# duckietown/gym-duckietown

Hardware: NVIDIA H100
Metric: env-steps/sec (obs+reward+done) at N envs, 1/2/4/8 H100 vs CPU ref (higher is better)
Workload: dtype f64 logic / f32 raster / u8 obs

## Files before the change

### gym-duckietown_b200/csrc/dts_render.cu

```cuda
#include <algorithm>
#include <cstddef>
#include <cstdlib>
#include <iterator>
#include <type_traits>
#include <utility>
#include <vector>

#include "dts_camera.cuh"
#include "dts_kernels.h"

namespace dts {

struct RemapTab {
  const int32_t* src_xy;
  const short4* cbox;
  const short4* fbox;
  const int32_t* cell_start;
  const uint16_t* cell_bins;
  const int32_t* home_start;
  const int4* home_ent;
  int ext_x, ext_y;
  const uint16_t* table_of_env;
  int count;
  const float2* fwd;
// ... 532 lines not shown
  }
  if (cls_out) *cls_out = 0;
  if (ltq & 0x00ff0000) {
    const unsigned ti = si.tex;
    const int lw = (ti >> 24) & 15, lh = ti >> 28;
    const int tw = 1 << lw, th = 1 << lh;
    const float twf = __int_as_float((127 + lw) << 23), thf = __int_as_float((127 + lh) << 23);
    const float tx = u * twf - 0.5f, ty = v * thf - 0.5f;
    const int txi = __float2int_rd(tx), tyi = __float2int_rd(ty);
    const float ffx = tx - (float)txi, ffy = ty - (float)tyi;
    const unsigned ti0 = (unsigned)txi & (tw - 1), ti1 = (ti0 + 1) & (tw - 1);
    const unsigned tj0 = (unsigned)tyi & (th - 1), tj1 = (tj0 + 1) & (th - 1);
    const unsigned r0 = tj0 << lw, r1 = tj1 << lw;
    const uchar4* tp = reinterpret_cast<const uchar4*>(tex_pool + ((size_t)(ti & 0xffffffu) << 8));
    const uchar4 t00 = __ldg(tp + (r0 + ti0)), t10 = __ldg(tp + (r0 + ti1));
    const uchar4 t01 = __ldg(tp + (r1 + ti0)), t11 = __ldg(tp + (r1 + ti1));
    const float a0[3] = {(float)t00.x, (float)t00.y, (float)t00.z}, a1[3] = {(float)t10.x, (float)t10.y, (float)t10.z};
    const float b0[3] = {(float)t01.x, (float)t01.y, (float)t01.z}, b1[3] = {(float)t11.x, (float)t11.y, (float)t11.z};
#pragma unroll
    for (int ch = 0; ch < 3; ch++) {
      const float ta = fmaf(ffx, a1[ch] - a0[ch], a0[ch]);
      const float tb = fmaf(ffx, b1[ch] - b0[ch], b0[ch]);
      const float tc = fmaf(ffy, tb - ta, ta);
      c3[ch] = tc * (c3[ch] * 0.00392156862745098f);
    }
    if (cls_out) {
      const unsigned cu = (unsigned)__float2int_rd(u * twf) & (tw - 1), cv = (unsigned)__float2int_rd(v * thf) & (th - 1);
      *cls_out = __ldg(cls_pool + ((size_t)(ti & 0xffffffu) << 6) + ((cv << lw) + cu));
    }
  }
}
__device__ __forceinline__ void shade_prim(const PrimRec* __restrict__ prims, unsigned w, const uint8_t* __restrict__ tex_pool,
                                           const float4* __restrict__ lat_tab, int pxa, int pya, float c3[3], float* qq_out = nullptr,
                                           const uint8_t* __restrict__ cls_pool = nullptr, int* cls_out = nullptr) {
  const ShadeIn si = load_shade(prims, w);
  shade_eval(si, tex_pool, lat_tab, pxa, pya, c3, qq_out, cls_pool, cls_out);
}

__device__ __forceinline__ uint32_t smem_u32(const void* p) { return (uint32_t)__cvta_generic_to_shared(p); }
__device__ __forceinline__ void mbar_init(uint64_t* bar, int count) {
  asm volatile("mbarrier.init.shared::cta.b64 [%0], %1;" ::"r"(smem_u32(bar)), "r"(count) : "memory");
}
__device__ __forceinline__ void mbar_fence_init() {
  asm volatile("fence.mbarrier_init.release.cluster;" ::: "memory");
  asm volatile("fence.proxy.async.shared::cta;" ::: "memory");
}
__device__ __forceinline__ void mbar_expect_tx(uint64_t* bar, uint32_t bytes) {
  asm volatile("mbarrier.arrive.expect_tx.shared::cta.b64 _, [%0], %1;" ::"r"(smem_u32(bar)), "r"(bytes) : "memory");
}
__device__ __forceinline__ void bulk_load(void* dst_smem, const void* src_gmem, uint32_t bytes, uint64_t* bar) {
  asm volatile("cp.async.bulk.shared::cluster.global.mbarrier::complete_tx::bytes [%0], [%1], %2, [%3];" ::"r"(smem_u32(dst_smem)),
               "l"(src_gmem), "r"(bytes), "r"(smem_u32(bar))
               : "memory");
}
__device__ __forceinline__ void mbar_wait(uint64_t* bar, uint32_t parity) {
  uint32_t ok;
  do {
    asm volatile("{\n .reg .pred p;\n mbarrier.try_wait.parity.shared::cta.b64 p, [%1], %2;\n selp.u32 %0, 1, 0, p;\n}"
                 : "=r"(ok)
                 : "r"(smem_u32(bar)), "r"(parity)
                 : "memory");
  } while (!ok);
}

__device__ __forceinline__ unsigned pack_rgb(float r, float g, float b) {
  const unsigned ur = min(__float2uint_rn(r * 255.0f), 255u);
  const unsigned ug = min(__float2uint_rn(g * 255.0f), 255u);
  const unsigned ub = min(__float2uint_rn(b * 255.0f), 255u);
  return ur | (ug << 8) | (ub << 16);
}

struct StoreLane {
  int src_lo, src_hi;
  int sh8;
  int off;
  int j, row;
};
__device__ __forceinline__ StoreLane make_store_lane(int lane, int W) {
  StoreLane sl;
  const int j = lane & 7, rowbase = lane & ~7;
  const int p0 = (4 * j) / 3;
  sl.sh8 = (4 * j - 3 * p0) * 8;
  sl.src_lo = rowbase + min(p0, 7);
  sl.src_hi = rowbase + min(p0 + 1, 7);
  sl.off = (lane >> 3) * W * 3 + 4 * j;
  sl.j = j; sl.row = lane >> 3;
  return sl;
}
__device__ __forceinline__ void store_bin_fast(uint8_t* __restrict__ bin0, const StoreLane& sl, unsigned rgb, int rows_ok) {
  const unsigned lo = __shfl_sync(0xffffffffu, rgb, sl.src_lo);
  const unsigned hi = __shfl_sync(0xffffffffu, rgb, sl.src_hi);
  const unsigned word = __funnelshift_r(lo | (hi << 24), hi >> 8, sl.sh8);
  if (sl.j < 6 && sl.row < rows_ok) *reinterpret_cast<unsigned*>(bin0 + sl.off) = word;
}
__device__ __forceinline__ void store_bin_bytes(uint8_t* __restrict__ out, unsigned rgb, int lane, int bx, int by, int W, int H) {
  const int gx = bx * kBinW + (lane & 7), gy = by * kBinH + (lane >> 3);
  if (gx < W && gy < H) {
    uint8_t* d = out + ((size_t)gy * W + gx) * 3;
    d[0] = (uint8_t)(rgb & 255); d[1] = (uint8_t)((rgb >> 8) & 255); d[2] = (uint8_t)(rgb >> 16);
  }
}

__device__ __forceinline__ unsigned fine_rows_in_image(int cby, int H) { return ((cby * kCFY + 1) * kBinH < H) ? 0xffu : 0x0fu; }
__device__ __forceinline__ unsigned fine_in_image(int cbx, unsigned rows, int W) {
  const int nx = min(kCFX, (W - cbx * kCoarseW + kBinW - 1) / kBinW);
  const unsigned cols = (1u << nx) - 1u;
// ... 642 lines not shown
  __syncthreads();
  BinRec* recs = fm.recs;
  for (int i = pair0 + tid; i < pair0 + total; i += nthr) {
    const uint32_t pair = pairs[i];
    const int p = (int)(pair & 0xffffu), b = (int)(pair >> 16);
    const int cby = b / cbins_x, cbx = b - cby * cbins_x;
    unsigned r;
    if (kRemap != kRemapNone) {
      const short4 cb = rt.cbox[b];
      r = build_binrec(prims + p, p, cb.x * kSub, cb.y * kSub, recs + i, rt.fbox + (size_t)b * 8);
    } else {
      r = build_binrec(prims + p, p, cbx * kCoarseW * kSub, cby * kCoarseH * kSub, recs + i);
    }
    const int c = cnt[b];
    const unsigned valid = fine_in_image(cbx, fine_rows_in_image(cby, H), W);
    const bool alone = (r & kRecGround) ? (c & kCountMask) == 1 : (c & kCountMask) - (c >> 20) == 1;
    if (alone && (r & valid) == valid) {
      fm.bin_count[(size_t)env * cbins + b] = -(p + 1);
      const int slot = atomicAdd(fm.work + kWorkSoloList, 1);
      fm.solo[slot] = make_uint2((unsigned)env, (unsigned)b | ((unsigned)p << 16));
      atomicOr(&no_flat[b], 1 | kSoloMark);
    }
    if (!(r & kRecFlatOk)) atomicOr(&no_flat[b], 1);
  }
  __syncthreads();
  for (int b0 = wib * 32; b0 < cbins; b0 += nthr) {
    const int b = b0 + lane, c = b < cbins ? (cnt[b] & kCountMask) : 0;
    const bool flat = c >= 1 && c <= kStage && !no_flat[b];
    const bool empty = kRemap == kRemapNone && (W & 3) == 0 && b < cbins && c == 0;
    const unsigned m = __ballot_sync(0xffffffffu, flat), me = __ballot_sync(0xffffffffu, empty);
    if (m) {
      int base = 0;
      if (lane == 0) base = atomicAdd(fm.work + kWorkFlatList, __popc(m));
      base = __shfl_sync(0xffffffffu, base, 0);
      if (flat) {
        fm.bin_count[(size_t)env * cbins + b] = kFlatBin;
        fm.flat[base + __popc(m & ((1u << lane) - 1u))] = make_uint2((unsigned)env, (unsigned)b | ((unsigned)c << 16));
      }
    }
    if (me) {
      DTS_COUNT(30, __popc(me));
      int base = 0;
      if (lane == 0) base = atomicAdd(fm.work + kWorkEmptyList, __popc(me));
      base = __shfl_sync(0xffffffffu, base, 0);
      if (empty) {
        fm.bin_count[(size_t)env * cbins + b] = kEmptyBin;
        fm.empty[base + __popc(me & ((1u << lane) - 1u))] = make_uint2((unsigned)env, (unsigned)b);
      }
    }
    if (b < cbins && (rc.all_rows || (!flat && !empty && !(no_flat[b] & kSoloMark)))) row_to_list(fm, env, b / cbins_x, cbins_y);
  }
}

__device__ __noinline__ void gather_rows_out(const uint8_t* __restrict__ src, const GatherTab& gt, size_t off, size_t nbytes, int lane) {
  __syncwarp();
  const uint8_t* s = src + off;
  if (((reinterpret_cast<size_t>(s) | nbytes) & 15) == 0) {
    bool aligned = true;
    for (int p = 0; p < gt.n; p++) aligned &= (reinterpret_cast<size_t>(gt.base[p] + off) & 15) == 0;
    if (aligned) {
      for (size_t i = (size_t)lane * 16; i < nbytes; i += 512) {
        const int4 v = __ldcg(reinterpret_cast<const int4*>(s + i));
        for (int p = 0; p < gt.n; p++) *reinterpret_cast<int4*>(gt.base[p] + off + i) = v;
      }
      return;
    }
  }
  for (size_t i = lane; i < nbytes; i += 32) {
    const uint8_t v = __ldcg(s + i);
    for (int p = 0; p < gt.n; p++) gt.base[p][off + i] = v;
  }
}

constexpr size_t kRasterSmem = (sizeof(BinRec) * 2 * kStage + 16 + 128 * sizeof(unsigned long long)) * kWarps;
__device__ __forceinline__ unsigned float_key(float f) { const unsigned b = __float_as_uint(f); return b ^ ((b >> 31) ? 0xffffffffu : 0x80000000u); }
__device__ __forceinline__ float key_float(unsigned k) { return __uint_as_float(k ^ ((k >> 31) ? 0x80000000u : 0xffffffffu)); }

__device__ __forceinline__ int sample_mask(const BinRec& br, int pxc, int pyc) {
  const int4 E = *reinterpret_cast<const int4*>(br.E0);
  const int4 A = *reinterpret_cast<const int4*>(br.A);
  const int4 B = *reinterpret_cast<const int4*>(br.B);
  const int ec0 = E.x + A.x * pxc + B.x * pyc;
  const int ec1 = E.y + A.y * pxc + B.y * pyc;
  const int ec2 = E.z + A.z * pxc + B.z * pyc;
  int mask = 0;
  if (br.kind & kKindQuad) {
    const int ec3 = E.w + A.w * pxc + B.w * pyc;
#pragma unroll
    for (int s = 0; s < 4; s++) {
      const int e0 = ec0 + A.x * sample_x(s) + B.x * sample_y(s);
      const int e1 = ec1 + A.y * sample_x(s) + B.y * sample_y(s);
      const int e2 = ec2 + A.z * sample_x(s) + B.z * sample_y(s);
      const int e3 = ec3 + A.w * sample_x(s) + B.w * sample_y(s);
      if ((e0 | e1 | e2 | e3) >= 0) mask |= 1 << s;
    }
  } else {
#pragma unroll
    for (int s = 0; s < 4; s++) {
      const int e0 = ec0 + A.x * sample_x(s) + B.x * sample_y(s);
      const int e1 = ec1 + A.y * sample_x(s) + B.y * sample_y(s);
      const int e2 = ec2 + A.z * sample_x(s) + B.z * sample_y(s);
      if ((e0 | e1 | e2) >= 0) mask |= 1 << s;
    }
  }
  return mask;
}

template <int kAux, typename LabelOf>
__device__ __forceinline__ void resolve_edge(const unsigned wn[4], float c3[3], const float clr[3], const PrimRec* __restrict__ prims,
                                             const uint8_t* __restrict__ tex_pool, const float4* __restrict__ lat_tab, int pxa, int pya,
                                             int lane, int32_t* __restrict__ err, AuxPx& pix, const LabelOf& label_of,
                                             const uint8_t* __restrict__ cls_pool) {
  (void)lane; (void)err;
  float s01[3] = {c3[0], c3[1], c3[2]}, s23[3] = {0.f, 0.f, 0.f};
  unsigned pend = 0xeu;
  if (wn[1] == wn[0]) { pend &= ~2u; s01[0] = s01[0] + c3[0]; s01[1] = s01[1] + c3[1]; s01[2] = s01[2] + c3[2]; }
#pragma unroll
  for (int t = 2; t < 4; t++)
    if (wn[t] == wn[0]) { pend &= ~(1u << t); s23[0] = s23[0] + c3[0]; s23[1] = s23[1] + c3[1]; s23[2] = s23[2] + c3[2]; }
#pragma unroll 1
  while (__any_sync(0xffffffffu, pend != 0u)) {
    DTS_COUNT(12, 1);
    if (pend) {
      const int s = __ffs(pend) - 1;
      const unsigned w = s == 1 ? wn[1] : (s == 2 ? wn[2] : wn[3]);
      float d3[3] = {clr[0], clr[1], clr[2]};
      float qq = 0.0f;
      int c = 0;
      if (w != kNoPrim)
        shade_prim(prims, w, tex_pool, lat_tab, pxa, pya, d3, needs_qq(kAux) ? &qq : nullptr, cls_pool,
                   (kAux & kAuxMarks) ? &c : nullptr);
      if (takes_winner(kAux)) {
        if (w != kNoPrim) take_winner<kAux>(pix, qq, w, c, label_of);
      } else if (kAux & kAuxDepth) {
        pix.qmax = fmaxf(pix.qmax, qq);
      }
#pragma unroll
      for (int t = 1; t < 4; t++)
        if ((pend >> t & 1u) && wn[t] == w) {
          pend &= ~(1u << t);
          if (t < 2) { s01[0] = s01[0] + d3[0]; s01[1] = s01[1] + d3[1]; s01[2] = s01[2] + d3[2]; }
          else { s23[0] = s23[0] + d3[0]; s23[1] = s23[1] + d3[1]; s23[2] = s23[2] + d3[2]; }
        }
    }
  }
#pragma unroll
  for (int ch = 0; ch < 3; ch++) c3[ch] = (s01[ch] + s23[ch]) * 0.25f;
}
template <int kAux, typename LabelOf>
__device__ __forceinline__ unsigned shade_resolve(const unsigned wn[4], bool simple, const float clr[3], const PrimRec* __restrict__ prims,
                                                  const uint8_t* __restrict__ tex_pool, const float4* __restrict__ lat_tab, int pxa,
                                                  int pya, int lane, int32_t* __restrict__ err, AuxPx& pix, const LabelOf& label_of,
                                                  const uint8_t* __restrict__ cls_pool) {
  const bool same = wn[1] == wn[0] && wn[2] == wn[0] && wn[3] == wn[0];
  const bool all_same = simple || __all_sync(0xffffffffu, same);
  float c3[3] = {clr[0], clr[1], clr[2]};
  pix = AuxPx{};
  if (wn[0] != kNoPrim) {
    shade_prim(prims, wn[0], tex_pool, lat_tab, pxa, pya, c3, needs_qq(kAux) ? &pix.qmax : nullptr, cls_pool,
               (kAux & kAuxMarks) ? &pix.mk : nullptr);
    if (takes_winner(kAux)) pix.lab = label_of(wn[0]);
  }
  if (!all_same)
    resolve_edge<kAux>(wn, c3, clr, prims, tex_pool, lat_tab, pxa, pya, lane, err, pix, label_of, cls_pool);
  return pack_rgb(c3[0], c3[1], c3[2]);
}

template <int kRemap, int kAux>
__global__ void __launch_bounds__(kThreads, kRasterMinCtas)
k_raster(const DState S, const DMap* __restrict__ maps, RenderCfg rc, FrameMem fm, RemapTab rts, GatherTab gt,
         uint8_t* __restrict__ obs, int max_prims, int max_pairs, int max_lat, int32_t* __restrict__ err, AuxTargets aux) {
  extern __shared__ __align__(128) unsigned char raster_smem[];
  BinRec (*stages)[2][kStage] = reinterpret_cast<BinRec (*)[2][kStage]>(raster_smem);
  uint64_t (*bars)[2] = reinterpret_cast<uint64_t (*)[2]>(raster_smem + sizeof(BinRec) * kWarps * 2 * kStage);
  unsigned long long* zb = reinterpret_cast<unsigned long long*>(raster_smem + sizeof(BinRec) * kWarps * 2 * kStage + 16 * kWarps) +
                           128 * (threadIdx.x >> 5);
  const int W = rc.width, H = rc.height;
  const int cbins_x = (W + kCoarseW - 1) / kCoarseW, cbins_y = (H + kCoarseH - 1) / kCoarseH, cbins = cbins_x * cbins_y;
  const int lane = threadIdx.x & 31, warp = threadIdx.x >> 5;
  const size_t frame_bytes = (size_t)W * H * 3;
  const int pxs = (lane & 7) * kSub, pys = (lane >> 3) * kSub;
  const StoreLane sl = make_store_lane(lane, W);
  uint64_t* bar = bars[warp];
  if (lane == 0) { mbar_init(&bar[0], 1); mbar_init(&bar[1], 1); mbar_fence_init(); }
  __syncwarp();
  uint32_t parity = 0;
  int cs = 0, ps = 0;
  const int n_work = fm.work[kWorkRowList];
  int work = 0;
  if (lane == 0) work = atomicAdd(fm.work + kWorkRaster, 1);
  work = __shfl_sync(0xffffffffu, work, 0);
  while (work < n_work) {
    int next_work = 0;
    if (lane == 0) next_work = atomicAdd(fm.work + kWorkRaster, 1);
    const uint2 row = fm.rows[work];
    const int env = (int)row.x, cby = (int)row.y;
    const RemapTab rt = kRemap == kRemapPool ? remap_of_env(rts, env, W, H, cbins) : rts;
    const DMap& m = maps[S.map_id[env]];
    const uint8_t* tex_pool = m.tex_pool;
    const PrimRec* prims = fm.prims + (size_t)env * max_prims;
    const BinRec* recs = fm.recs;
    const float4* lat_tab = fm.lat + (size_t)env * max_lat * 64;
    const size_t env_off = (size_t)env * frame_bytes;
    uint8_t* out = obs + env_off;
    const AuxFrames af = aux_frames(aux, env, W, H);
    const uint8_t* cls_pool = (kAux & kAuxMarks) ? tex_pool + m.tex_class_off : nullptr;
    LabelMap lm{};
    if constexpr (takes_winner(kAux)) lm = label_map(m, rc.tessellate);
    auto label_of = [&](unsigned w) { return label_of_id(lm, __ldg(&prims[w].id)); };
    auto emit = [&](unsigned rgb, float depth, int label, int mark, int bx, int by) {
      store_aux<kAux>(af, depth, label, mark, lane, bx, by, W, H);
      store_bin(out, sl, rgb, lane, bx, by, W, H);
    };
    float clr[3];
    clear_colour(S, rc, env, clr);
    const unsigned clear_rgb = pack_rgb(clr[0], clr[1], clr[2]);
    int my_cnt = 0, my_start = 0;
    if (lane < cbins_x) {
      my_cnt = fm.bin_count[(size_t)env * cbins + cby * cbins_x + lane];
      my_start = fm.bin_start[(size_t)env * cbins + cby * cbins_x + lane];
    }
    const unsigned nz = __ballot_sync(0xffffffffu, my_cnt > 0);
    int pcbx = nz ? __ffs(nz) - 1 : 32, pf = 0, pc = 0;
    const unsigned rows_in = fine_rows_in_image(cby, H);
    auto fine_valid = [&](int cbx, int f) -> bool { return (fine_in_image(cbx, rows_in, W) >> f) & 1u; };
    auto next_bin = [&]() {
      const unsigned rem = nz & ~((2u << pcbx) - 1u);
      pcbx = rem ? __ffs(rem) - 1 : 32;
      pf = 0; pc = 0;
    };
    auto issue = [&]() {
      if (pcbx >= 32) return;
      const int n = __shfl_sync(0xffffffffu, my_cnt, pcbx), st = __shfl_sync(0xffffffffu, my_start, pcbx);
      if (n > kStage) while (pf < kCFX * kCFY && !fine_valid(pcbx, pf)) pf++;
      if (n > kStage && pf >= kCFX * kCFY) { next_bin(); return; }
      const int nch = min(kStage, n - pc);
      if (lane == 0) {
        mbar_expect_tx(&bar[ps], (uint32_t)(nch * sizeof(BinRec)));
        bulk_load(stages[warp][ps], recs + st + pc, (uint32_t)(nch * sizeof(BinRec)), &bar[ps]);
      }
      ps ^= 1;
      if (n <= kStage) { next_bin(); return; }
      pc += kStage;
      if (pc >= n) {
        pc = 0; pf++;
        while (pf < kCFX * kCFY && !fine_valid(pcbx, pf)) pf++;
        if (pf >= kCFX * kCFY) next_bin();
      }
    };
    issue();
    for (int cbx = 0; cbx < cbins_x; cbx++) {
      const int count = __shfl_sync(0xffffffffu, my_cnt, cbx);
      if (count < 0) continue;
      const unsigned fvalid = fine_in_image(cbx, rows_in, W);
      DTS_COUNT(8, 1);
      if (count == 0) {
        DTS_COUNT(9, 1);
#pragma unroll 1
        for (int f = 0; f < kCFX * kCFY; f++)
          if ((fvalid >> f) & 1u) {
            const int bx = cbx * kCFX + (f & 3), by = cby * kCFY + (f >> 2);
            unsigned rgb = clear_rgb;
            if (kRemap != kRemapNone && !remap_source(rt, bx, by, lane, W, H).valid) rgb = 0u;
            emit(rgb, 0.0f, 0, 0, bx, by);
          }
        continue;
      }
      const bool single = count <= kStage;
      DTS_COUNT(10, count);
      if (!single) { DTS_COUNT(14, 1); DTS_COUNT(15, count); }
      int ox = cbx * kCoarseW * kSub, oy = cby * kCoarseH * kSub;
      if (kRemap != kRemapNone) { const short4 cb = rt.cbox[cby * cbins_x + cbx]; ox = cb.x * kSub; oy = cb.y * kSub; }
#pragma unroll 1
      for (int g = 0; g < (single ? 1 : kCFX * kCFY); g++) {
        if (!single && !((fvalid >> g) & 1u)) continue;
        float z[4];
        unsigned wn[4];
        bool zb_used = false;
#pragma unroll 1
        for (int c0 = 0; c0 < count; c0 += kStage) {
          __syncwarp();
          issue();
          mbar_wait(&bar[cs], (parity >> cs) & 1u);
          parity ^= 1u << cs;
          const BinRec* stage = stages[warp][cs];
          cs ^= 1;
          const int nch = min(kStage, count - c0);
          uint2 mine = make_uint2(0u, 0u);
          if (lane < nch) mine = *reinterpret_cast<const uint2*>(&stage[lane].prim_flags);
          const bool first = c0 == 0, last = c0 + kStage >= count;
          const unsigned ground_bits = __ballot_sync(0xffffffffu, (mine.y & kKindGround) != 0u);
          const unsigned tiny_bits = kRemap != kRemapNone ? 0u : __ballot_sync(0xffffffffu, (mine.y & kKindTiny) != 0u);
          const unsigned flat_bits = __ballot_sync(0xffffffffu, (mine.y & kKindFlat) != 0u);
#if DTS_STATS
          if (single) {
            const unsigned ng_ = __ballot_sync(0xffffffffu, !(mine.y & kKindGround) && ((mine.x >> 16) & fvalid) != 0u);
            const unsigned ngfull_ = __ballot_sync(0xffffffffu, !(mine.y & kKindGround) && ((mine.x >> 24) & fvalid) == fvalid);
            if (ng_ && !(ng_ & (ng_ - 1)) && (ng_ & ngfull_)) { DTS_COUNT(22, 1); DTS_COUNT(23, __popc(fvalid)); }
          }
#endif
#pragma unroll 1
          for (int f = (single ? 0 : g); f < (single ? kCFX * kCFY : g + 1); f++) {
            if (!((fvalid >> f) & 1u)) continue;
            const int bx = cbx * kCFX + (f & 3), by = cby * kCFY + (f >> 2);
            int pxc = pxs + (f & 3) * kBinW * kSub, pyc = pys + (f >> 2) * kBinH * kSub;
            bool px_valid = true;
            if (kRemap != kRemapNone) {
              const RemapPx src = remap_source(rt, bx, by, lane, W, H);
              px_valid = src.valid;
              pxc = src.x - ox; pyc = src.y - oy;
            }
            const bool live = (mine.x >> (16 + f)) & 1u;
            const unsigned live_mask = __ballot_sync(0xffffffffu, live);
            const unsigned ground_mask = live_mask & ground_bits;
            bool simple = false;
            if (single) {
              const unsigned full_mask = __ballot_sync(0xffffffffu, live && ((mine.x >> (24 + f)) & 1u));
              const unsigned others = live_mask & ~ground_mask;
              const unsigned pick = others ? others : live_mask;
              if (pick && !(pick & (pick - 1)) && (pick & full_mask)) {
                simple = true;
                DTS_COUNT(13, 1);
                const unsigned w = stage[__ffs(pick) - 1].prim_flags & 0xffffu;
                wn[0] = w; wn[1] = w; wn[2] = w; wn[3] = w;
              }
            }
            bool coplanar = single && !(live_mask & ~ground_mask & ~flat_bits);
            if (coplanar && !simple) DTS_COUNT(20, 1);
            if (!simple) {
              if (first) {
#pragma unroll
                for (int s = 0; s < 4; s++) { z[s] = 1.0f; wn[s] = kNoPrim; }
                zb_used = false;
              }
#pragma unroll 1
              for (int phase = 0; phase < 2; phase++) {
                unsigned todo = phase == 0 ? (live_mask & ~ground_mask & ~tiny_bits) : ground_mask;
                if (phase == 1 && todo &&
                    __all_sync(0xffffffffu, wn[0] != kNoPrim && wn[1] != kNoPrim && wn[2] != kNoPrim && wn[3] != kNoPrim))
                  todo = 0;
                int seen = 0, twice = 0;
                while (todo) {
                  const int k = __ffs(todo) - 1;
                  todo &= todo - 1;
                  const BinRec& br = stage[k];
                  const uint32_t pflags = br.prim_flags;
                  DTS_COUNT(16, 1);
                  if ((pflags >> (24 + f)) & 1u) DTS_COUNT(17, 1);
                  int mask = 15;
                  if (!((pflags >> (24 + f)) & 1u)) {
                    mask = sample_mask(br, pxc, pyc);
                    if (!mask) continue;
                  }
                  if (coplanar && phase == 0) {
                    twice |= seen & mask;
                    seen |= mask;
#pragma unroll
                    for (int s = 0; s < 4; s++)
                      if (mask >> s & 1) wn[s] = pflags & 0xffffu;
                    continue;
                  }
                  const float4 zp = *reinterpret_cast<const float4*>(&br.z0);
                  const int2 xy0 = *reinterpret_cast<const int2*>(&br.x0);
                  const float cdx = (float)(pxc + 32 - xy0.x) * 0.015625f, cdy = (float)(pyc + 32 - xy0.y) * 0.015625f;
                  float zs[4];
                  int lt = 0, eq = 0;
#pragma unroll
                  for (int s = 0; s < 4; s++) {
                    const float sdx = cdx + (float)(sample_x(s) - 32) * 0.015625f, sdy = cdy + (float)(sample_y(s) - 32) * 0.015625f;
                    zs[s] = fmaf(zp.z, sdy, fmaf(zp.y, sdx, zp.x));
                    lt |= (zs[s] < z[s]) << s;
                    eq |= (zs[s] == z[s]) << s;
                  }
                  int pass_mask = mask & lt;
                  const int tie = mask & eq;
                  if (tie) {
                    const int my_id = __float_as_int(zp.w);
#pragma unroll
                    for (int s = 0; s < 4; s++)
                      if ((tie >> s & 1) && wn[s] != kNoPrim && my_id < __ldg(&prims[wn[s]].id)) pass_mask |= 1 << s;
                  }
                  if (!pass_mask) continue;
                  const unsigned me = pflags & 0xffffu;
#pragma unroll
                  for (int s = 0; s < 4; s++)
                    if (pass_mask >> s & 1) { z[s] = zs[s]; wn[s] = me; }
                }
                if (coplanar && phase == 0) {
                  if (__any_sync(0xffffffffu, twice != 0)) {
                    coplanar = false;
                    DTS_COUNT(21, 1);
#pragma unroll
                    for (int s = 0; s < 4; s++) wn[s] = kNoPrim;
                    phase = -1;
                  } else {
#pragma unroll
                    for (int s = 0; s < 4; s++)
                      if (seen >> s & 1) z[s] = -1.0f;
                  }
                }
              }
            }
            if (kRemap == kRemapNone && !simple && (live_mask & tiny_bits)) {
              if (!zb_used) {
                zb_used = true;
#pragma unroll
                for (int s = 0; s < 4; s++) zb[lane * 4 + s] = ~0ull;
                __syncwarp();
              }
              DTS_COUNT(18, 1);
              DTS_COUNT(19, __popc(live_mask & tiny_bits));
              if ((live_mask & tiny_bits) >> lane & 1u) {
                const BinRec& br = stage[lane];
                const int4 E = *reinterpret_cast<const int4*>(br.E0);
                const int4 A = *reinterpret_cast<const int4*>(br.A);
                const int4 B = *reinterpret_cast<const int4*>(br.B);
                const float4 zp = *reinterpret_cast<const float4*>(&br.z0);
                const int2 xy0 = *reinterpret_cast<const int2*>(&br.x0);
                const int fx0 = (f & 3) * kBinW, fy0 = (f >> 2) * kBinH;
                const int x_lo = max(E.w & 0xffff, fx0), x_hi = min(A.w & 0xffff, fx0 + kBinW - 1);
                const int y_lo = max(E.w >> 16, fy0), y_hi = min(A.w >> 16, fy0 + kBinH - 1);
                const unsigned long long tail = ((unsigned long long)(unsigned)__float_as_int(zp.w) << 16) | (br.prim_flags & 0xffffu);
                for (int py = y_lo; py <= y_hi; py++)
                  for (int px = x_lo; px <= x_hi; px++) {
                    const int X = px * kSub, Y = py * kSub;
                    const int ec0 = E.x + A.x * X + B.x * Y, ec1 = E.y + A.y * X + B.y * Y, ec2 = E.z + A.z * X + B.z * Y;
#pragma unroll
                    for (int s = 0; s < 4; s++) {
                      const int e0 = ec0 + A.x * sample_x(s) + B.x * sample_y(s);
                      const int e1 = ec1 + A.y * sample_x(s) + B.y * sample_y(s);
                      const int e2 = ec2 + A.z * sample_x(s) + B.z * sample_y(s);
                      if ((e0 | e1 | e2) < 0) continue;
                      const float sdx = (float)(X + sample_x(s) - xy0.x) * 0.015625f, sdy = (float)(Y + sample_y(s) - xy0.y) * 0.015625f;
                      const float zs = fmaf(zp.z, sdy, fmaf(zp.y, sdx, zp.x));
                      atomicMin(&zb[((py - fy0) * kBinW + (px - fx0)) * 4 + s], ((unsigned long long)float_key(zs) << 32) | tail);
                    }
                  }
              }
              __syncwarp();
            }
            if (!(last || simple)) continue;
            if (kRemap == kRemapNone && !simple && zb_used) {
#pragma unroll
              for (int s = 0; s < 4; s++) {
                const unsigned long long k = zb[lane * 4 + s];
                if (k == ~0ull) continue;
                const float zt = key_float((unsigned)(k >> 32));
                bool win = zt < z[s];
                if (zt == z[s] && wn[s] != kNoPrim) win = (int)((k >> 16) & 0xffffu) < __ldg(&prims[wn[s]].id);
                if (win) { z[s] = zt; wn[s] = (unsigned)(k & 0xffffu); }
              }
              __syncwarp();
            }
            DTS_COUNT(11, 1);
            AuxPx pix;
            unsigned rgb = shade_resolve<kAux>(wn, simple, clr, prims, tex_pool, lat_tab, ox + pxc, oy + pyc, lane, err, pix,
                                               label_of, cls_pool);
            if (kRemap != kRemapNone && !px_valid) rgb = 0u;
            emit(rgb, depth_of(pix.qmax, px_valid), px_valid ? pix.lab : 0, px_valid ? pix.mk : 0, bx, by);
          }
        }
      }
    }
    if (gt.n > 0) {
      const int rows = min(kCoarseH, H - cby * kCoarseH);
      gather_rows_out(obs, gt, env_off + (size_t)cby * kCoarseH * W * 3, (size_t)rows * W * 3, lane);
    }
    work = __shfl_sync(0xffffffffu, next_work, 0);
  }
}

template <int kAux>
__device__ __forceinline__ void clear_empty_bins(const DState& S, const RenderCfg& rc, const FrameMem& fm, uint8_t* __restrict__ obs,
                                                 const AuxTargets& aux) {
  constexpr int kBatch = 8;
  const int W = rc.width, H = rc.height;
  const int cbins_x = (W + kCoarseW - 1) / kCoarseW;
  const int lane = threadIdx.x & 31, n = fm.work[kWorkEmptyList];
  const int warps = (gridDim.x * blockDim.x) >> 5;
  for (int i0 = ((blockIdx.x * blockDim.x + threadIdx.x) >> 5) * kBatch; i0 < n; i0 += warps * kBatch) {
    uint2 e = make_uint2(0u, 0u);
    unsigned rgb = 0u;
    if (lane < kBatch && i0 + lane < n) {
      e = fm.empty[i0 + lane];
      float clr[3];
      clear_colour(S, rc, (int)e.x, clr);
      rgb = pack_rgb(clr[0], clr[1], clr[2]);
    }
#pragma unroll 1
    for (int j = 0; j < min(kBatch, n - i0); j++) {
      const int env = (int)__shfl_sync(0xffffffffu, e.x, j), b = (int)__shfl_sync(0xffffffffu, e.y, j);
      const unsigned c = __shfl_sync(0xffffffffu, rgb, j);
      const int cby = b / cbins_x, x0 = (b - cby * cbins_x) * kCoarseW;
      const int px = min(kCoarseW, W - x0), rows = min(kCoarseH, H - cby * kCoarseH);
      const int k3 = lane % 3;
      const unsigned word = k3 == 0 ? (c | (c << 24)) : (k3 == 1 ? ((c >> 8) | (c << 16)) : ((c >> 16) | (c << 8)));
      const size_t pix0 = (size_t)env * W * H + (size_t)(cby * kCoarseH) * W + x0;
#pragma unroll 1
      for (int r = 0; r < rows; r++) {
        const size_t pix = pix0 + (size_t)r * W;
        if (lane < px * 3 / 4) reinterpret_cast<unsigned*>(obs + pix * 3)[lane] = word;
        if (lane < px) {
          if (stores_depth<kAux>(aux.depth)) aux.depth[pix + lane] = 0.0f;
          if (kAux & kAuxLabels) aux.labels[pix + lane] = 0;
          if (kAux & kAuxMarks) aux.marks[pix + lane] = 0;
        }
      }
    }
  }
}

template <int kRemap, int kAux>
__global__ void __launch_bounds__(kThreads, kSoloMinCtas) k_raster_solo(const DState S, const DMap* __restrict__ maps, RenderCfg rc, FrameMem fm,
                                                                        RemapTab rts, uint8_t* __restrict__ obs, int max_prims, int max_lat,
                                                                        AuxTargets aux) {
  const int W = rc.width, H = rc.height;
  const int cbins_x = (W + kCoarseW - 1) / kCoarseW;
  const int lane = threadIdx.x & 31;
  const StoreLane sl = make_store_lane(lane, W);
  const size_t frame_bytes = (size_t)W * H * 3;
  if (kRemap == kRemapNone) clear_empty_bins<kAux>(S, rc, fm, obs, aux);
// ... 522 lines not shown
```

Measured before the change: 2.823 million.

## Share coarse-row work across CTA with one warp per fine bin and shared TMA ring

Changes k_raster so a whole CTA claims a coarse row and each warp handles one fine bin, instead of each warp independently processing a full row and looping over all 16 fine bins. Warp 0 produces bulk async loads into a shared 8-slot ring guarded by full/empty mbarriers, and all warps consume the same staged BinRec chunks, so each chunk is loaded once per CTA rather than repeatedly per warp. The row gather is spread over all CTA threads. This adds __syncthreads per row and producer/consumer coupling. Warps with invalid or empty fine bins idle or only step through the ring, so uneven per-bin work can leave warps waiting on each other.

```diff
diff --git a/gym-duckietown_b200/csrc/dts_render.cu b/gym-duckietown_b200/csrc/dts_render.cu
--- a/gym-duckietown_b200/csrc/dts_render.cu
+++ b/gym-duckietown_b200/csrc/dts_render.cu
@@ -608,6 +608,17 @@
   asm volatile("cp.async.bulk.shared::cluster.global.mbarrier::complete_tx::bytes [%0], [%1], %2, [%3];" ::"r"(smem_u32(dst_smem)),
                "l"(src_gmem), "r"(bytes), "r"(smem_u32(bar))
                : "memory");
+}
+__device__ __forceinline__ void mbar_arrive(uint64_t* bar) {
+  asm volatile("mbarrier.arrive.shared::cta.b64 _, [%0];" ::"r"(smem_u32(bar)) : "memory");
+}
+__device__ __forceinline__ bool mbar_test(uint64_t* bar, uint32_t parity) {
+  uint32_t ok;
+  asm volatile("{\n .reg .pred p;\n mbarrier.test_wait.parity.shared::cta.b64 p, [%1], %2;\n selp.u32 %0, 1, 0, p;\n}"
+               : "=r"(ok)
+               : "r"(smem_u32(bar)), "r"(parity)
+               : "memory");
+  return ok != 0u;
 }
 __device__ __forceinline__ void mbar_wait(uint64_t* bar, uint32_t parity) {
   uint32_t ok;
@@ -1356,27 +1367,28 @@
   }
 }
 
-__device__ __noinline__ void gather_rows_out(const uint8_t* __restrict__ src, const GatherTab& gt, size_t off, size_t nbytes, int lane) {
-  __syncwarp();
+__device__ __noinline__ void gather_rows_out(const uint8_t* __restrict__ src, const GatherTab& gt, size_t off, size_t nbytes, int tid,
+                                             int nthr) {
   const uint8_t* s = src + off;
   if (((reinterpret_cast<size_t>(s) | nbytes) & 15) == 0) {
     bool aligned = true;
     for (int p = 0; p < gt.n; p++) aligned &= (reinterpret_cast<size_t>(gt.base[p] + off) & 15) == 0;
     if (aligned) {
-      for (size_t i = (size_t)lane * 16; i < nbytes; i += 512) {
+      for (size_t i = (size_t)tid * 16; i < nbytes; i += (size_t)nthr * 16) {
         const int4 v = __ldcg(reinterpret_cast<const int4*>(s + i));
         for (int p = 0; p < gt.n; p++) *reinterpret_cast<int4*>(gt.base[p] + off + i) = v;
       }
       return;
     }
   }
-  for (size_t i = lane; i < nbytes; i += 32) {
+  for (size_t i = tid; i < nbytes; i += nthr) {
     const uint8_t v = __ldcg(s + i);
     for (int p = 0; p < gt.n; p++) gt.base[p][off + i] = v;
   }
 }
 
-constexpr size_t kRasterSmem = (sizeof(BinRec) * 2 * kStage + 16 + 128 * sizeof(unsigned long long)) * kWarps;
+constexpr int kRing = 8;
+constexpr size_t kRasterSmem = sizeof(BinRec) * kRing * kStage + 2 * kRing * sizeof(uint64_t) + 128 * sizeof(unsigned long long) * kWarps;
 __device__ __forceinline__ unsigned float_key(float f) { const unsigned b = __float_as_uint(f); return b ^ ((b >> 31) ? 0xffffffffu : 0x80000000u); }
 __device__ __forceinline__ float key_float(unsigned k) { return __uint_as_float(k ^ ((k >> 31) ? 0x80000000u : 0xffffffffu)); }
 
@@ -1470,33 +1482,37 @@
   return pack_rgb(c3[0], c3[1], c3[2]);
 }
 
+static_assert(kWarps == kCFX * kCFY, "k_raster: one warp per fine bin of a coarse bin");
 template <int kRemap, int kAux>
 __global__ void __launch_bounds__(kThreads, kRasterMinCtas)
 k_raster(const DState S, const DMap* __restrict__ maps, RenderCfg rc, FrameMem fm, RemapTab rts, GatherTab gt,
          uint8_t* __restrict__ obs, int max_prims, int max_pairs, int max_lat, int32_t* __restrict__ err, AuxTargets aux) {
   extern __shared__ __align__(128) unsigned char raster_smem[];
-  BinRec (*stages)[2][kStage] = reinterpret_cast<BinRec (*)[2][kStage]>(raster_smem);
-  uint64_t (*bars)[2] = reinterpret_cast<uint64_t (*)[2]>(raster_smem + sizeof(BinRec) * kWarps * 2 * kStage);
-  unsigned long long* zb = reinterpret_cast<unsigned long long*>(raster_smem + sizeof(BinRec) * kWarps * 2 * kStage + 16 * kWarps) +
-                           128 * (threadIdx.x >> 5);
+  __shared__ int row_claim[2];
+  BinRec (*ring)[kStage] = reinterpret_cast<BinRec (*)[kStage]>(raster_smem);
+  uint64_t* full = reinterpret_cast<uint64_t*>(raster_smem + sizeof(BinRec) * kRing * kStage);
+  uint64_t* empty = full + kRing;
+  unsigned long long* zb = reinterpret_cast<unsigned long long*>(empty + kRing) + 128 * (threadIdx.x >> 5);
   const int W = rc.width, H = rc.height;
   const int cbins_x = (W + kCoarseW - 1) / kCoarseW, cbins_y = (H + kCoarseH - 1) / kCoarseH, cbins = cbins_x * cbins_y;
   const int lane = threadIdx.x & 31, warp = threadIdx.x >> 5;
+  const int f = warp;
   const size_t frame_bytes = (size_t)W * H * 3;
   const int pxs = (lane & 7) * kSub, pys = (lane >> 3) * kSub;
   const StoreLane sl = make_store_lane(lane, W);
-  uint64_t* bar = bars[warp];
-  if (lane == 0) { mbar_init(&bar[0], 1); mbar_init(&bar[1], 1); mbar_fence_init(); }
-  __syncwarp();
-  uint32_t parity = 0;
-  int cs = 0, ps = 0;
+  if (threadIdx.x == 0) {
+    for (int s = 0; s < kRing; s++) { mbar_init(&full[s], 1); mbar_init(&empty[s], kWarps); }
+    mbar_fence_init();
+  }
+  uint32_t q = 0;
+  uint32_t issued = 0;
   const int n_work = fm.work[kWorkRowList];
-  int work = 0;
-  if (lane == 0) work = atomicAdd(fm.work + kWorkRaster, 1);
-  work = __shfl_sync(0xffffffffu, work, 0);
+  if (threadIdx.x == 0) row_claim[0] = atomicAdd(fm.work + kWorkRaster, 1);
+  __syncthreads();
+  int slot = 0, work = row_claim[0];
   while (work < n_work) {
     int next_work = 0;
-    if (lane == 0) next_work = atomicAdd(fm.work + kWorkRaster, 1);
+    if (threadIdx.x == 0) next_work = atomicAdd(fm.work + kWorkRaster, 1);
     const uint2 row = fm.rows[work];
     const int env = (int)row.x, cby = (int)row.y;
     const RemapTab rt = kRemap == kRemapPool ? remap_of_env(rts, env, W, H, cbins) : rts;
@@ -1519,258 +1535,265 @@
     float clr[3];
     clear_colour(S, rc, env, clr);
     const unsigned clear_rgb = pack_rgb(clr[0], clr[1], clr[2]);
+    const unsigned rows_in = fine_rows_in_image(cby, H);
     int my_cnt = 0, my_start = 0;
     if (lane < cbins_x) {
       my_cnt = fm.bin_count[(size_t)env * cbins + cby * cbins_x + lane];
       my_start = fm.bin_start[(size_t)env * cbins + cby * cbins_x + lane];
     }
-    const unsigned nz = __ballot_sync(0xffffffffu, my_cnt > 0);
-    int pcbx = nz ? __ffs(nz) - 1 : 32, pf = 0, pc = 0;
-    const unsigned rows_in = fine_rows_in_image(cby, H);
-    auto fine_valid = [&](int cbx, int f) -> bool { return (fine_in_image(cbx, rows_in, W) >> f) & 1u; };
-    auto next_bin = [&]() {
-      const unsigned rem = nz & ~((2u << pcbx) - 1u);
-      pcbx = rem ? __ffs(rem) - 1 : 32;
-      pf = 0; pc = 0;
+    const unsigned staged = __ballot_sync(0xffffffffu, my_cnt > 0);
+    int pcbx = staged ? __ffs(staged) - 1 : 32, pc = 0;
+    auto produce = [&](bool need) {
+      while (pcbx < 32 && issued < q + kRing) {
+        const int s = (int)(issued % kRing);
+        const uint32_t u = issued / kRing;
+        if (u > 0) {
+          if (need && issued == q) mbar_wait(&empty[s], (u - 1u) & 1u);
+          else if (!__shfl_sync(0xffffffffu, (int)mbar_test(&empty[s], (u - 1u) & 1u), 0)) break;
+        }
+        const int n = __shfl_sync(0xffffffffu, my_cnt, pcbx), st = __shfl_sync(0xffffffffu, my_start, pcbx);
+        const int nch = min(kStage, n - pc);
+        if (lane == 0) {
+          mbar_expect_tx(&full[s], (uint32_t)(nch * sizeof(BinRec)));
+          bulk_load(ring[s], recs + st + pc, (uint32_t)(nch * sizeof(BinRec)), &full[s]);
+        }
+        issued++;
+        pc += kStage;
+        if (pc >= n) {
+          const unsigned rem = staged & ~((2u << pcbx) - 1u);
+          pcbx = rem ? __ffs(rem) - 1 : 32;
+          pc = 0;
+        }
+      }
     };
-    auto issue = [&]() {
-      if (pcbx >= 32) return;
-      const int n = __shfl_sync(0xffffffffu, my_cnt, pcbx), st = __shfl_sync(0xffffffffu, my_start, pcbx);
-      if (n > kStage) while (pf < kCFX * kCFY && !fine_valid(pcbx, pf)) pf++;
-      if (n > kStage && pf >= kCFX * kCFY) { next_bin(); return; }
-      const int nch = min(kStage, n - pc);
-      if (lane == 0) {
-        mbar_expect_tx(&bar[ps], (uint32_t)(nch * sizeof(BinRec)));
-        bulk_load(stages[warp][ps], recs + st + pc, (uint32_t)(nch * sizeof(BinRec)), &bar[ps]);
-      }
-      ps ^= 1;
-      if (n <= kStage) { next_bin(); return; }
-      pc += kStage;
-      if (pc >= n) {
-        pc = 0; pf++;
-        while (pf < kCFX * kCFY && !fine_valid(pcbx, pf)) pf++;
-        if (pf >= kCFX * kCFY) next_bin();
-      }
+    bool held = false;
+    auto release = [&]() {
+      __syncwarp();
+      if (held && lane == 0) mbar_arrive(&empty[(q - 1u) % kRing]);
+      held = false;
     };
-    issue();
+    auto acquire = [&]() -> const BinRec* {
+      release();
+      if (warp == 0) produce(true);
+      const int s = (int)(q % kRing);
+      mbar_wait(&full[s], (q / kRing) & 1u);
+      held = true;
+      q++;
+      return ring[s];
+    };
+    if (warp == 0) produce(false);
     for (int cbx = 0; cbx < cbins_x; cbx++) {
       const int count = __shfl_sync(0xffffffffu, my_cnt, cbx);
       if (count < 0) continue;
       const unsigned fvalid = fine_in_image(cbx, rows_in, W);
-      DTS_COUNT(8, 1);
+      const bool drawn = (fvalid >> f) & 1u;
+      if (!drawn) {
+        for (int c0 = 0; c0 < count; c0 += kStage) acquire();
+        continue;
+      }
+      const int bx = cbx * kCFX + (f & 3), by = cby * kCFY + (f >> 2);
+      if (warp == 0) DTS_COUNT(8, 1);
       if (count == 0) {
-        DTS_COUNT(9, 1);
-#pragma unroll 1
-        for (int f = 0; f < kCFX * kCFY; f++)
-          if ((fvalid >> f) & 1u) {
-            const int bx = cbx * kCFX + (f & 3), by = cby * kCFY + (f >> 2);
-            unsigned rgb = clear_rgb;
-            if (kRemap != kRemapNone && !remap_source(rt, bx, by, lane, W, H).valid) rgb = 0u;
-            emit(rgb, 0.0f, 0, 0, bx, by);
-          }
+        if (warp == 0) DTS_COUNT(9, 1);
+        unsigned rgb = clear_rgb;
+        if (kRemap != kRemapNone && !remap_source(rt, bx, by, lane, W, H).valid) rgb = 0u;
+        emit(rgb, 0.0f, 0, 0, bx, by);
         continue;
       }
       const bool single = count <= kStage;
-      DTS_COUNT(10, count);
-      if (!single) { DTS_COUNT(14, 1); DTS_COUNT(15, count); }
+      if (warp == 0) {
+        DTS_COUNT(10, count);
+        if (!single) { DTS_COUNT(14, 1); DTS_COUNT(15, count); }
+      }
       int ox = cbx * kCoarseW * kSub, oy = cby * kCoarseH * kSub;
       if (kRemap != kRemapNone) { const short4 cb = rt.cbox[cby * cbins_x + cbx]; ox = cb.x * kSub; oy = cb.y * kSub; }
+      float z[4];
+      unsigned wn[4];
+      bool zb_used = false;
 #pragma unroll 1
-      for (int g = 0; g < (single ? 1 : kCFX * kCFY); g++) {
-        if (!single && !((fvalid >> g) & 1u)) continue;
-        float z[4];
-        unsigned wn[4];
-        bool zb_used = false;
+      for (int c0 = 0; c0 < count; c0 += kStage) {
+        const BinRec* stage = acquire();
+        const int nch = min(kStage, count - c0);
+        uint2 mine = make_uint2(0u, 0u);
+        if (lane < nch) mine = *reinterpret_cast<const uint2*>(&stage[lane].prim_flags);
+        const bool first = c0 == 0, last = c0 + kStage >= count;
+        const unsigned ground_bits = __ballot_sync(0xffffffffu, (mine.y & kKindGround) != 0u);
+        const unsigned tiny_bits = kRemap != kRemapNone ? 0u : __ballot_sync(0xffffffffu, (mine.y & kKindTiny) != 0u);
+        const unsigned flat_bits = __ballot_sync(0xffffffffu, (mine.y & kKindFlat) != 0u);
+#if DTS_STATS
+        if (single && warp == 0) {
+          const unsigned ng_ = __ballot_sync(0xffffffffu, !(mine.y & kKindGround) && ((mine.x >> 16) & fvalid) != 0u);
+          const unsigned ngfull_ = __ballot_sync(0xffffffffu, !(mine.y & kKindGround) && ((mine.x >> 24) & fvalid) == fvalid);
+          if (ng_ && !(ng_ & (ng_ - 1)) && (ng_ & ngfull_)) { DTS_COUNT(22, 1); DTS_COUNT(23, __popc(fvalid)); }
+        }
+#endif
+        int pxc = pxs + (f & 3) * kBinW * kSub, pyc = pys + (f >> 2) * kBinH * kSub;
+        bool px_valid = true;
+        if (kRemap != kRemapNone) {
+          const RemapPx src = remap_source(rt, bx, by, lane, W, H);
+          px_valid = src.valid;
+          pxc = src.x - ox; pyc = src.y - oy;
+        }
+        const bool live = (mine.x >> (16 + f)) & 1u;
+        const unsigned live_mask = __ballot_sync(0xffffffffu, live);
+        const unsigned ground_mask = live_mask & ground_bits;
+        bool simple = false;
+        if (single) {
+          const unsigned full_mask = __ballot_sync(0xffffffffu, live && ((mine.x >> (24 + f)) & 1u));
+          const unsigned others = live_mask & ~ground_mask;
+          const unsigned pick = others ? others : live_mask;
+          if (pick && !(pick & (pick - 1)) && (pick & full_mask)) {
+            simple = true;
+            DTS_COUNT(13, 1);
+            const unsigned w = stage[__ffs(pick) - 1].prim_flags & 0xffffu;
+            wn[0] = w; wn[1] = w; wn[2] = w; wn[3] = w;
+          }
+        }
+        bool coplanar = single && !(live_mask & ~ground_mask & ~flat_bits);
+        if (coplanar && !simple) DTS_COUNT(20, 1);
+        if (!simple) {
+          if (first) {
+#pragma unroll
+            for (int s = 0; s < 4; s++) { z[s] = 1.0f; wn[s] = kNoPrim; }
+            zb_used = false;
+          }
 #pragma unroll 1
-        for (int c0 = 0; c0 < count; c0 += kStage) {
-          __syncwarp();
-          issue();
-          mbar_wait(&bar[cs], (parity >> cs) & 1u);
-          parity ^= 1u << cs;
-          const BinRec* stage = stages[warp][cs];
-          cs ^= 1;
-          const int nch = min(kStage, count - c0);
-          uint2 mine = make_uint2(0u, 0u);
-          if (lane < nch) mine = *reinterpret_cast<const uint2*>(&stage[lane].prim_flags);
-          const bool first = c0 == 0, last = c0 + kStage >= count;
-          const unsigned ground_bits = __ballot_sync(0xffffffffu, (mine.y & kKindGround) != 0u);
-          const unsigned tiny_bits = kRemap != kRemapNone ? 0u : __ballot_sync(0xffffffffu, (mine.y & kKindTiny) != 0u);
-          const unsigned flat_bits = __ballot_sync(0xffffffffu, (mine.y & kKindFlat) != 0u);
-#if DTS_STATS
-          if (single) {
-            const unsigned ng_ = __ballot_sync(0xffffffffu, !(mine.y & kKindGround) && ((mine.x >> 16) & fvalid) != 0u);
-            const unsigned ngfull_ = __ballot_sync(0xffffffffu, !(mine.y & kKindGround) && ((mine.x >> 24) & fvalid) == fvalid);
-            if (ng_ && !(ng_ & (ng_ - 1)) && (ng_ & ngfull_)) { DTS_COUNT(22, 1); DTS_COUNT(23, __popc(fvalid)); }
-          }
-#endif
-#pragma unroll 1
-          for (int f = (single ? 0 : g); f < (single ? kCFX * kCFY : g + 1); f++) {
-            if (!((fvalid >> f) & 1u)) continue;
-            const int bx = cbx * kCFX + (f & 3), by = cby * kCFY + (f >> 2);
-            int pxc = pxs + (f & 3) * kBinW * kSub, pyc = pys + (f >> 2) * kBinH * kSub;
-            bool px_valid = true;
-            if (kRemap != kRemapNone) {
-              const RemapPx src = remap_source(rt, bx, by, lane, W, H);
-              px_valid = src.valid;
-              pxc = src.x - ox; pyc = src.y - oy;
+          for (int phase = 0; phase < 2; phase++) {
+            unsigned todo = phase == 0 ? (live_mask & ~ground_mask & ~tiny_bits) : ground_mask;
+            if (phase == 1 && todo &&
+                __all_sync(0xffffffffu, wn[0] != kNoPrim && wn[1] != kNoPrim && wn[2] != kNoPrim && wn[3] != kNoPrim))
+              todo = 0;
+            int seen = 0, twice = 0;
+            while (todo) {
+              const int k = __ffs(todo) - 1;
+              todo &= todo - 1;
+              const BinRec& br = stage[k];
+              const uint32_t pflags = br.prim_flags;
+              DTS_COUNT(16, 1);
+              if ((pflags >> (24 + f)) & 1u) DTS_COUNT(17, 1);
+              int mask = 15;
+              if (!((pflags >> (24 + f)) & 1u)) {
+                mask = sample_mask(br, pxc, pyc);
+                if (!mask) continue;
+              }
+              if (coplanar && phase == 0) {
+                twice |= seen & mask;
+                seen |= mask;
+#pragma unroll
+                for (int s = 0; s < 4; s++)
+                  if (mask >> s & 1) wn[s] = pflags & 0xffffu;
+                continue;
+              }
+              const float4 zp = *reinterpret_cast<const float4*>(&br.z0);
+              const int2 xy0 = *reinterpret_cast<const int2*>(&br.x0);
+              const float cdx = (float)(pxc + 32 - xy0.x) * 0.015625f, cdy = (float)(pyc + 32 - xy0.y) * 0.015625f;
+              float zs[4];
+              int lt = 0, eq = 0;
+#pragma unroll
+              for (int s = 0; s < 4; s++) {
+                const float sdx = cdx + (float)(sample_x(s) - 32) * 0.015625f, sdy = cdy + (float)(sample_y(s) - 32) * 0.015625f;
+                zs[s] = fmaf(zp.z, sdy, fmaf(zp.y, sdx, zp.x));
+                lt |= (zs[s] < z[s]) << s;
+                eq |= (zs[s] == z[s]) << s;
+              }
+              int pass_mask = mask & lt;
+              const int tie = mask & eq;
+              if (tie) {
+                const int my_id = __float_as_int(zp.w);
+#pragma unroll
+                for (int s = 0; s < 4; s++)
+                  if ((tie >> s & 1) && wn[s] != kNoPrim && my_id < __ldg(&prims[wn[s]].id)) pass_mask |= 1 << s;
+              }
+              if (!pass_mask) continue;
+              const unsigned me = pflags & 0xffffu;
+#pragma unroll
+              for (int s = 0; s < 4; s++)
+                if (pass_mask >> s & 1) { z[s] = zs[s]; wn[s] = me; }
             }
-            const bool live = (mine.x >> (16 + f)) & 1u;
-            const unsigned live_mask = __ballot_sync(0xffffffffu, live);
-            const unsigned ground_mask = live_mask & ground_bits;
-            bool simple = false;
-            if (single) {
-              const unsigned full_mask = __ballot_sync(0xffffffffu, live && ((mine.x >> (24 + f)) & 1u));
-              const unsigned others = live_mask & ~ground_mask;
-              const unsigned pick = others ? others : live_mask;
-              if (pick && !(pick & (pick - 1)) && (pick & full_mask)) {
-                simple = true;
-                DTS_COUNT(13, 1);
-                const unsigned w = stage[__ffs(pick) - 1].prim_flags & 0xffffu;
-                wn[0] = w; wn[1] = w; wn[2] = w; wn[3] = w;
+            if (coplanar && phase == 0) {
+              if (__any_sync(0xffffffffu, twice != 0)) {
+                coplanar = false;
+                DTS_COUNT(21, 1);
+#pragma unroll
+                for (int s = 0; s < 4; s++) wn[s] = kNoPrim;
+                phase = -1;
+              } else {
+#pragma unroll
+                for (int s = 0; s < 4; s++)
+                  if (seen >> s & 1) z[s] = -1.0f;
               }
             }
-            bool coplanar = single && !(live_mask & ~ground_mask & ~flat_bits);
-            if (coplanar && !simple) DTS_COUNT(20, 1);
-            if (!simple) {
-              if (first) {
-#pragma unroll
-                for (int s = 0; s < 4; s++) { z[s] = 1.0f; wn[s] = kNoPrim; }
-                zb_used = false;
-              }
-#pragma unroll 1
-              for (int phase = 0; phase < 2; phase++) {
-                unsigned todo = phase == 0 ? (live_mask & ~ground_mask & ~tiny_bits) : ground_mask;
-                if (phase == 1 && todo &&
-                    __all_sync(0xffffffffu, wn[0] != kNoPrim && wn[1] != kNoPrim && wn[2] != kNoPrim && wn[3] != kNoPrim))
-                  todo = 0;
-                int seen = 0, twice = 0;
-                while (todo) {
-                  const int k = __ffs(todo) - 1;
-                  todo &= todo - 1;
-                  const BinRec& br = stage[k];
-                  const uint32_t pflags = br.prim_flags;
-                  DTS_COUNT(16, 1);
-                  if ((pflags >> (24 + f)) & 1u) DTS_COUNT(17, 1);
-                  int mask = 15;
-                  if (!((pflags >> (24 + f)) & 1u)) {
-                    mask = sample_mask(br, pxc, pyc);
-                    if (!mask) continue;
-                  }
-                  if (coplanar && phase == 0) {
-                    twice |= seen & mask;
-                    seen |= mask;
-#pragma unroll
-                    for (int s = 0; s < 4; s++)
-                      if (mask >> s & 1) wn[s] = pflags & 0xffffu;
-                    continue;
-                  }
-                  const float4 zp = *reinterpret_cast<const float4*>(&br.z0);
-                  const int2 xy0 = *reinterpret_cast<const int2*>(&br.x0);
-                  const float cdx = (float)(pxc + 32 - xy0.x) * 0.015625f, cdy = (float)(pyc + 32 - xy0.y) * 0.015625f;
-                  float zs[4];
-                  int lt = 0, eq = 0;
-#pragma unroll
-                  for (int s = 0; s < 4; s++) {
-                    const float sdx = cdx + (float)(sample_x(s) - 32) * 0.015625f, sdy = cdy + (float)(sample_y(s) - 32) * 0.015625f;
-                    zs[s] = fmaf(zp.z, sdy, fmaf(zp.y, sdx, zp.x));
-                    lt |= (zs[s] < z[s]) << s;
-                    eq |= (zs[s] == z[s]) << s;
-                  }
-                  int pass_mask = mask & lt;
-                  const int tie = mask & eq;
-                  if (tie) {
-                    const int my_id = __float_as_int(zp.w);
-#pragma unroll
-                    for (int s = 0; s < 4; s++)
-                      if ((tie >> s & 1) && wn[s] != kNoPrim && my_id < __ldg(&prims[wn[s]].id)) pass_mask |= 1 << s;
-                  }
-                  if (!pass_mask) continue;
-                  const unsigned me = pflags & 0xffffu;
-#pragma unroll
-                  for (int s = 0; s < 4; s++)
-                    if (pass_mask >> s & 1) { z[s] = zs[s]; wn[s] = me; }
-                }
-                if (coplanar && phase == 0) {
-                  if (__any_sync(0xffffffffu, twice != 0)) {
-                    coplanar = false;
-                    DTS_COUNT(21, 1);
-#pragma unroll
-                    for (int s = 0; s < 4; s++) wn[s] = kNoPrim;
-                    phase = -1;
-                  } else {
-#pragma unroll
-                    for (int s = 0; s < 4; s++)
-                      if (seen >> s & 1) z[s] = -1.0f;
-                  }
+          }
+        }
+        if (kRemap == kRemapNone && !simple && (live_mask & tiny_bits)) {
+          if (!zb_used) {
+            zb_used = true;
+#pragma unroll
+            for (int s = 0; s < 4; s++) zb[lane * 4 + s] = ~0ull;
+            __syncwarp();
+          }
+          DTS_COUNT(18, 1);
+          DTS_COUNT(19, __popc(live_mask & tiny_bits));
+          if ((live_mask & tiny_bits) >> lane & 1u) {
+            const BinRec& br = stage[lane];
+            const int4 E = *reinterpret_cast<const int4*>(br.E0);
+            const int4 A = *reinterpret_cast<const int4*>(br.A);
+            const int4 B = *reinterpret_cast<const int4*>(br.B);
+            const float4 zp = *reinterpret_cast<const float4*>(&br.z0);
+            const int2 xy0 = *reinterpret_cast<const int2*>(&br.x0);
+            const int fx0 = (f & 3) * kBinW, fy0 = (f >> 2) * kBinH;
+            const int x_lo = max(E.w & 0xffff, fx0), x_hi = min(A.w & 0xffff, fx0 + kBinW - 1);
+            const int y_lo = max(E.w >> 16, fy0), y_hi = min(A.w >> 16, fy0 + kBinH - 1);
+            const unsigned long long tail = ((unsigned long long)(unsigned)__float_as_int(zp.w) << 16) | (br.prim_flags & 0xffffu);
+            for (int py = y_lo; py <= y_hi; py++)
+              for (int px = x_lo; px <= x_hi; px++) {
+                const int X = px * kSub, Y = py * kSub;
+                const int ec0 = E.x + A.x * X + B.x * Y, ec1 = E.y + A.y * X + B.y * Y, ec2 = E.z + A.z * X + B.z * Y;
+#pragma unroll
+                for (int s = 0; s < 4; s++) {
+                  const int e0 = ec0 + A.x * sample_x(s) + B.x * sample_y(s);
+                  const int e1 = ec1 + A.y * sample_x(s) + B.y * sample_y(s);
+                  const int e2 = ec2 + A.z * sample_x(s) + B.z * sample_y(s);
+                  if ((e0 | e1 | e2) < 0) continue;
+                  const float sdx = (float)(X + sample_x(s) - xy0.x) * 0.015625f, sdy = (float)(Y + sample_y(s) - xy0.y) * 0.015625f;
+                  const float zs = fmaf(zp.z, sdy, fmaf(zp.y, sdx, zp.x));
+                  atomicMin(&zb[((py - fy0) * kBinW + (px - fx0)) * 4 + s], ((unsigned long long)float_key(zs) << 32) | tail);
                 }
               }
-            }
-            if (kRemap == kRemapNone && !simple && (live_mask & tiny_bits)) {
-              if (!zb_used) {
-                zb_used = true;
-#pragma unroll
-                for (int s = 0; s < 4; s++) zb[lane * 4 + s] = ~0ull;
-                __syncwarp();
-              }
-              DTS_COUNT(18, 1);
-              DTS_COUNT(19, __popc(live_mask & tiny_bits));
-              if ((live_mask & tiny_bits) >> lane & 1u) {
-                const BinRec& br = stage[lane];
-                const int4 E = *reinterpret_cast<const int4*>(br.E0);
-                const int4 A = *reinterpret_cast<const int4*>(br.A);
-                const int4 B = *reinterpret_cast<const int4*>(br.B);
-                const float4 zp = *reinterpret_cast<const float4*>(&br.z0);
-                const int2 xy0 = *reinterpret_cast<const int2*>(&br.x0);
-                const int fx0 = (f & 3) * kBinW, fy0 = (f >> 2) * kBinH;
-                const int x_lo = max(E.w & 0xffff, fx0), x_hi = min(A.w & 0xffff, fx0 + kBinW - 1);
-                const int y_lo = max(E.w >> 16, fy0), y_hi = min(A.w >> 16, fy0 + kBinH - 1);
-                const unsigned long long tail = ((unsigned long long)(unsigned)__float_as_int(zp.w) << 16) | (br.prim_flags & 0xffffu);
-                for (int py = y_lo; py <= y_hi; py++)
-                  for (int px = x_lo; px <= x_hi; px++) {
-                    const int X = px * kSub, Y = py * kSub;
-                    const int ec0 = E.x + A.x * X + B.x * Y, ec1 = E.y + A.y * X + B.y * Y, ec2 = E.z + A.z * X + B.z * Y;
-#pragma unroll
-                    for (int s = 0; s < 4; s++) {
-                      const int e0 = ec0 + A.x * sample_x(s) + B.x * sample_y(s);
-                      const int e1 = ec1 + A.y * sample_x(s) + B.y * sample_y(s);
-                      const int e2 = ec2 + A.z * sample_x(s) + B.z * sample_y(s);
-                      if ((e0 | e1 | e2) < 0) continue;
-                      const float sdx = (float)(X + sample_x(s) - xy0.x) * 0.015625f, sdy = (float)(Y + sample_y(s) - xy0.y) * 0.015625f;
-                      const float zs = fmaf(zp.z, sdy, fmaf(zp.y, sdx, zp.x));
-                      atomicMin(&zb[((py - fy0) * kBinW + (px - fx0)) * 4 + s], ((unsigned long long)float_key(zs) << 32) | tail);
-                    }
-                  }
-              }
-              __syncwarp();
-            }
-            if (!(last || simple)) continue;
-            if (kRemap == kRemapNone && !simple && zb_used) {
-#pragma unroll
-              for (int s = 0; s < 4; s++) {
-                const unsigned long long k = zb[lane * 4 + s];
-                if (k == ~0ull) continue;
-                const float zt = key_float((unsigned)(k >> 32));
-                bool win = zt < z[s];
-                if (zt == z[s] && wn[s] != kNoPrim) win = (int)((k >> 16) & 0xffffu) < __ldg(&prims[wn[s]].id);
-                if (win) { z[s] = zt; wn[s] = (unsigned)(k & 0xffffu); }
-              }
-              __syncwarp();
-            }
-            DTS_COUNT(11, 1);
-            AuxPx pix;
-            unsigned rgb = shade_resolve<kAux>(wn, simple, clr, prims, tex_pool, lat_tab, ox + pxc, oy + pyc, lane, err, pix,
-                                               label_of, cls_pool);
-            if (kRemap != kRemapNone && !px_valid) rgb = 0u;
-            emit(rgb, depth_of(pix.qmax, px_valid), px_valid ? pix.lab : 0, px_valid ? pix.mk : 0, bx, by);
           }
+          __syncwarp();
         }
-      }
-    }
+        if (!(last || simple)) continue;
+        if (kRemap == kRemapNone && !simple && zb_used) {
+#pragma unroll
+          for (int s = 0; s < 4; s++) {
+            const unsigned long long k = zb[lane * 4 + s];
+            if (k == ~0ull) continue;
+            const float zt = key_float((unsigned)(k >> 32));
+            bool win = zt < z[s];
+            if (zt == z[s] && wn[s] != kNoPrim) win = (int)((k >> 16) & 0xffffu) < __ldg(&prims[wn[s]].id);
+            if (win) { z[s] = zt; wn[s] = (unsigned)(k & 0xffffu); }
+          }
+          __syncwarp();
+        }
+        DTS_COUNT(11, 1);
+        AuxPx pix;
+        unsigned rgb = shade_resolve<kAux>(wn, simple, clr, prims, tex_pool, lat_tab, ox + pxc, oy + pyc, lane, err, pix,
+                                           label_of, cls_pool);
+        if (kRemap != kRemapNone && !px_valid) rgb = 0u;
+        emit(rgb, depth_of(pix.qmax, px_valid), px_valid ? pix.lab : 0, px_valid ? pix.mk : 0, bx, by);
+      }
+    }
+    release();
     if (gt.n > 0) {
+      __syncthreads();
       const int rows = min(kCoarseH, H - cby * kCoarseH);
-      gather_rows_out(obs, gt, env_off + (size_t)cby * kCoarseH * W * 3, (size_t)rows * W * 3, lane);
-    }
-    work = __shfl_sync(0xffffffffu, next_work, 0);
+      gather_rows_out(obs, gt, env_off + (size_t)cby * kCoarseH * W * 3, (size_t)rows * W * 3, threadIdx.x, kThreads);
+    }
+    slot ^= 1;
+    if (threadIdx.x == 0) row_claim[slot] = next_work;
+    __syncthreads();
+    work = row_claim[slot];
   }
 }
 
```

Result: faster. 2.903 million, median of 6 (+2.8%).
